# geekieo/collaborative-deep-metric-learning

Measured on NVIDIA B200. Metric: train_triplets_per_sec, higher is better.
Workload: dtype fp16 operands / fp32 accumulate (tcgen05 kind::f16), fp32 master weights

## Files before the change

collaborative-deep-metric-learning_b200/_lib.py:

```python
import ctypes
import os
from ctypes import POINTER, c_char_p, c_float, c_int, c_int32, c_int64, c_void_p

_HERE = os.path.dirname(os.path.abspath(__file__))
LIB_PATH = os.path.join(_HERE, "libcdml.so")

F16, BF16 = 0, 1
EPI_STORE_F32, EPI_STORE_16, EPI_L2NORM, EPI_MASK_LEAKY, EPI_MASK_BITS = 0, 1, 2, 3, 4
METRIC_L2, METRIC_IP = 0, 1

_P = c_void_p
_SIGNATURES = {
  "cdml_ctx_create": (c_int, [c_int, POINTER(c_void_p)]),
  "cdml_ctx_destroy": (c_int, [_P]),
  "cdml_last_error": (c_char_p, []),
  "cdml_version": (c_int, []),
  "cdml_ctx_poll_errors": (c_int, [_P, _P, POINTER(c_int32)]),
  "cdml_gather_rows": (c_int, [_P, _P, c_int64, c_int64, c_int64, _P, c_int, c_int64, _P, c_int64, _P]),
  "cdml_rows_normalize_cast": (c_int, [_P, _P, c_int64, c_int64, c_int64, c_int, c_float, _P, c_int64, c_int, _P,
                                       c_int64, _P, _P]),
  "cdml_gemm16": (c_int, [_P, _P, c_int, c_int64, _P, c_int, c_int64, c_int64, c_int64, c_int64, c_int, c_int, _P,
                          c_int64, _P, c_float, _P, _P, c_int64, c_int, c_int64, POINTER(c_int), _P]),
  "cdml_gemm16_auto_splits": (c_int, [_P, c_int64, c_int64, c_int64]),
  "cdml_sum_partials": (c_int, [_P, _P, c_int, c_int64, c_int64, c_float, _P, _P]),
  "cdml_colsum_workspace_floats": (c_int64, [c_int64, c_int64]),
  "cdml_colsum16": (c_int, [_P, _P, c_int64, c_int64, c_int64, c_int, _P, _P, _P]),
  "cdml_triplet_hinge": (c_int, [_P, _P, c_int64, c_int, c_int64, _P, c_float, c_float, _P, c_float, _P, _P, _P, _P,
                                 _P, _P, c_int64, c_int, _P, _P]),
  "cdml_adam_prepare": (c_int, [_P, _P, c_float, c_float, c_float, c_int, c_float, c_float, _P, _P]),
  "cdml_adam_apply": (c_int, [_P, _P, _P, _P, _P, c_int64, _P, c_float, c_float, c_float, c_float, _P, c_int, _P]),
  "cdml_opt_workspace_floats": (c_int64, []),
  "cdml_opt_sumsq": (c_int, [_P, _P, _P, c_int64, c_float, c_float, _P, _P, _P]),
  "cdml_opt_apply": (c_int, [_P, c_int, _P, _P, _P, _P, c_int64, _P, _P, c_float, c_float, c_float, c_float, c_float,
                             c_float, c_float, c_float, c_float, _P, c_int, _P]),
  "cdml_ew16": (c_int, [_P, c_int, _P, c_int64, _P, c_int64, _P, c_int64, _P, c_int64, c_int64, c_int, c_float, c_int, _P]),
  "cdml_rows_l2norm16": (c_int, [_P, _P, c_int64, c_int, c_int64, c_float, c_int, _P, c_int64, _P, _P, c_int64, _P]),
  "cdml_desim_workspace_bytes": (c_int64, [c_int64, c_int, c_int]),
  "cdml_desim": (c_int, [_P, _P, c_int64, c_int, c_int64, _P, _P, c_int64, c_int, c_int64, c_int64, c_float, c_int, _P, _P,
                         c_int64, c_int64, _P]),
  "cdml_desim_simple": (c_int, [_P, _P, c_int64, c_int, c_int64, _P, c_int, c_int64, _P, c_int64, _P]),
  "cdml_sample_triplets": (c_int, [_P, _P, c_int64, c_int64, c_int64, c_int64, ctypes.c_uint64, _P, _P]),
  "cdml_format_knn_rows": (c_int64, [_P, _P, c_int64, c_int, c_int64, c_int64, _P, _P, c_int64, _P, c_int64]),
  "cdml_format_f32": (c_int64, [_P, c_int64, _P, c_int64]),
  "cdml_parse_features_txt": (c_int64, [_P, c_int64, c_int, _P, c_int64, _P, _P, c_int]),
  "cdml_cast16": (c_int, [_P, _P, c_int64, _P, c_int, _P]),
  "cdml_fill_column16": (c_int, [_P, _P, c_int64, c_int64, c_int64, c_float, c_int, _P]),
  "cdml_mine_semihard": (c_int, [_P, _P, c_int64, c_int, _P, c_int64, _P, c_int64, c_int, c_float, _P, _P, _P]),
  "cdml_mine_distance_weighted": (c_int, [_P, _P, c_int64, c_int, _P, c_int64, _P, c_int64, c_int, c_float, c_float,
                                          ctypes.c_uint64, _P, _P, _P, _P]),
  "cdml_mine_last_stats": (c_int, [_P, _P, _P]),
  "cdml_knn_index_build": (c_int, [_P, _P, c_int64, c_int, c_int64, c_int, _P, POINTER(c_void_p)]),
  "cdml_knn_index_destroy": (c_int, [_P]),
  "cdml_knn_search": (c_int, [_P, _P, _P, c_int64, c_int64, c_int, _P, _P, c_int64, _P]),
  "cdml_knn_bounds": (c_int, [_P, _P, _P, c_int64, c_int64, c_int, c_int, _P, _P, _P]),
  "cdml_knn_search_bounded": (c_int, [_P, _P, _P, c_int64, c_int64, c_int, _P, _P, _P, _P, c_int64, _P]),
  "cdml_knn_last_stats": (c_int, [_P, POINTER(c_int64)]),
  "cdml_knn_merge": (c_int, [_P, _P, _P, c_int, c_int64, c_int, c_int, _P, _P, _P]),
  "cdml_knn_shard_bounds": (c_int, [_P, _P, _P, c_int64, c_int64, c_int, c_int, _P, _P]),
  "cdml_knn_shard_collect": (c_int, [_P, _P, _P, c_int64, c_int64, c_int, c_int, _P, _P, _P]),
  "cdml_knn_shard_refine": (c_int, [_P, _P, _P, c_int64, c_int64, c_int, _P, _P, c_int64, _P, _P]),
  "cdml_knn_merge_packed": (c_int, [_P, _P, c_int, c_int64, c_int, c_int, _P, _P, _P, _P]),
  "cdml_knn_unpack_records": (c_int, [_P, _P, c_int64, c_int, _P, _P, _P]),
  "cdml_mean_pair_dist": (c_int, [_P, _P, c_int64, c_int, _P, c_int64, _P, _P]),
# ... 56 lines not shown
```

collaborative-deep-metric-learning_b200/csrc/rowops.cu:

```cuda
#include <algorithm>
#include "../../include/cdml.h"
#include "ctx.cuh"

namespace cdml {

constexpr int kWarpsPerBlock = 8;
constexpr int kRowThreads = kWarpsPerBlock * 32;

__device__ __forceinline__ float warp_sum(float v) {
#pragma unroll
  for (int o = 16; o > 0; o >>= 1) v += __shfl_xor_sync(0xffffffffu, v, o);
  return v;
}

static inline int row_grid(cdml_ctx* ctx, int64_t rows) {
  const int64_t blocks = (rows + kWarpsPerBlock - 1) / kWarpsPerBlock;
  const int64_t cap = static_cast<int64_t>(ctx->num_sms) * 8;
  return static_cast<int>(blocks < cap ? (blocks > 0 ? blocks : 1) : cap);
}

template <typename IdxT, typename VecT>
__global__ void __launch_bounds__(kRowThreads)
gather_rows_kernel(const uint8_t* __restrict__ table, int64_t num_rows, int64_t row_bytes, int64_t pitch,
                   const IdxT* __restrict__ idx, int64_t n, uint8_t* __restrict__ out, int64_t out_pitch,
// ... 312 lines not shown
  __syncthreads();
  {
    float t = 0.f;
#pragma unroll
    for (int w = 0; w < kWarpsPerBlock; ++w) t += sh[w][threadIdx.x];
    const int64_t c = static_cast<int64_t>(blockIdx.x) * kColStripV + threadIdx.x;
    if (c < N) partial[static_cast<int64_t>(blockIdx.y) * N + c] = t;
  }
}

__global__ void sum_partials_kernel(const float* __restrict__ parts, int num_parts, int64_t stride, int64_t n,
                                    float scale, float* __restrict__ out) {
  for (int64_t i = static_cast<int64_t>(blockIdx.x) * blockDim.x + threadIdx.x; i < n;
       i += static_cast<int64_t>(gridDim.x) * blockDim.x) {
    float t = 0.f;
    for (int s = 0; s < num_parts; ++s) t += parts[s * stride + i];
    out[i] = t * scale;
  }
}

__global__ void sum_partials_vec4_kernel(const float4* __restrict__ parts, int num_parts, int64_t stride4, int64_t n4,
                                         float scale, float4* __restrict__ out) {
  for (int64_t i = static_cast<int64_t>(blockIdx.x) * blockDim.x + threadIdx.x; i < n4;
       i += static_cast<int64_t>(gridDim.x) * blockDim.x) {
    float4 t = make_float4(0.f, 0.f, 0.f, 0.f);
    for (int s = 0; s < num_parts; ++s) {
      const float4 v = __ldg(parts + s * stride4 + i);
      t.x += v.x, t.y += v.y, t.z += v.z, t.w += v.w;
    }
    out[i] = make_float4(t.x * scale, t.y * scale, t.z * scale, t.w * scale);
  }
}

__global__ void adam_prepare_kernel(int64_t* step, float base_lr, float decay_steps, float decay_rate, int staircase,
                                    float beta1, float beta2, float* scalars) {
  const int64_t gs = *step;
  const double t = static_cast<double>(gs + 1);
  double p = static_cast<double>(gs) / static_cast<double>(decay_steps);
  if (staircase) p = floor(p);
  const double lr = static_cast<double>(base_lr) * pow(static_cast<double>(decay_rate), p);
  const double lr_t = lr * sqrt(1.0 - pow(static_cast<double>(beta2), t)) / (1.0 - pow(static_cast<double>(beta1), t));
  scalars[0] = static_cast<float>(lr_t);
  scalars[1] = static_cast<float>(lr);
  scalars[2] = static_cast<float>(t);
  scalars[3] = 0.f;
  *step = gs + 1;
}

template <int kBf16>
__global__ void adam_apply_kernel(float* __restrict__ w, float* __restrict__ m, float* __restrict__ v,
                                  const float* __restrict__ g, int64_t n, const float* __restrict__ scalars,
                                  float beta1, float beta2, float eps, float gscale, uint16_t* __restrict__ w16) {
  const float lr_t = scalars[0];
  for (int64_t i = static_cast<int64_t>(blockIdx.x) * blockDim.x + threadIdx.x; i < n;
       i += static_cast<int64_t>(gridDim.x) * blockDim.x) {
    const float gi = g[i] * gscale;
    const float mi = beta1 * m[i] + (1.f - beta1) * gi;
    const float vi = beta2 * v[i] + (1.f - beta2) * gi * gi;
    const float wi = w[i] - lr_t * mi / (sqrtf(vi) + eps);
    m[i] = mi, v[i] = vi, w[i] = wi;
    if (w16 != nullptr) w16[i] = static_cast<uint16_t>(pack2<kBf16>(wi, 0.f));
  }
}

__global__ void fill_column16_kernel(uint16_t* __restrict__ X, int64_t rows, int64_t ld, int64_t col, uint16_t bits) {
  for (int64_t r = static_cast<int64_t>(blockIdx.x) * blockDim.x + threadIdx.x; r < rows;
       r += static_cast<int64_t>(gridDim.x) * blockDim.x)
    X[r * ld + col] = bits;
}

template <int kBf16>
__global__ void cast16_kernel(const float* __restrict__ in, int64_t n, uint16_t* __restrict__ out) {
  for (int64_t i = static_cast<int64_t>(blockIdx.x) * blockDim.x + threadIdx.x; i < n;
       i += static_cast<int64_t>(gridDim.x) * blockDim.x)
    out[i] = static_cast<uint16_t>(pack2<kBf16>(in[i], 0.f));
}

__global__ void __launch_bounds__(kRowThreads)
pair_dist_kernel(const float* __restrict__ V, int64_t ld, int D, const int64_t* __restrict__ pairs, int64_t P,
                 float* __restrict__ dist) {
  const int warp = threadIdx.x >> 5, lane = threadIdx.x & 31;
  for (int64_t i = static_cast<int64_t>(blockIdx.x) * kWarpsPerBlock + warp; i < P;
       i += static_cast<int64_t>(gridDim.x) * kWarpsPerBlock) {
    const float* a = V + pairs[2 * i] * ld;
    const float* b = V + pairs[2 * i + 1] * ld;
    float s = 0.f;
    for (int j = lane; j < D; j += 32) {
      const float d = a[j] - b[j];
      s = fmaf(d, d, s);
    }
    s = warp_sum(s);
    if (lane == 0) dist[i] = s;
  }
}
// ... 296 lines not shown
                                                                         stride / 4, n / 4, scale,
                                                                         reinterpret_cast<float4*>(out));
  else
    sum_partials_kernel<<<flat_grid(ctx, n, 256), 256, 0, st>>>(parts, num_parts, stride, n, scale, out);
  CDML_CHECK_CUDA(cudaGetLastError());
  return 0;
}

int cdml_adam_prepare(cdml_ctx* ctx, int64_t* step_counter, float base_lr, float decay_steps, float decay_rate,
                      int staircase, float beta1, float beta2, float* scalars, void* stream) {
  CDML_REQUIRE(ctx && step_counter && scalars, "cdml_adam_prepare: NULL argument");
  adam_prepare_kernel<<<1, 1, 0, static_cast<cudaStream_t>(stream)>>>(step_counter, base_lr, decay_steps, decay_rate,
                                                                      staircase, beta1, beta2, scalars);
  CDML_CHECK_CUDA(cudaGetLastError());
  return 0;
}

int cdml_adam_apply(cdml_ctx* ctx, float* w, float* m, float* v, const float* g, int64_t n, const float* scalars,
                    float beta1, float beta2, float eps, float grad_scale, void* w16, int dtype16, void* stream) {
  CDML_REQUIRE(ctx && w && m && v && g && scalars, "cdml_adam_apply: NULL argument");
  if (n == 0) return 0;
  cudaStream_t st = static_cast<cudaStream_t>(stream);
  const int grid = flat_grid(ctx, n, 256);
  if (dtype16 == CDML_BF16)
    adam_apply_kernel<1><<<grid, 256, 0, st>>>(w, m, v, g, n, scalars, beta1, beta2, eps, grad_scale,
                                               static_cast<uint16_t*>(w16));
  else
    adam_apply_kernel<0><<<grid, 256, 0, st>>>(w, m, v, g, n, scalars, beta1, beta2, eps, grad_scale,
                                               static_cast<uint16_t*>(w16));
  CDML_CHECK_CUDA(cudaGetLastError());
  return 0;
}

int64_t cdml_opt_workspace_floats(void) { return 2 * kSumsqBlocks + 2; }

int cdml_opt_sumsq(cdml_ctx* ctx, const float* g, const float* w, int64_t n, float grad_scale, float wd_reg,
                   float* workspace, float* out2, void* stream) {
  CDML_REQUIRE(ctx && g && w && workspace && out2 && n >= 0, "cdml_opt_sumsq: bad argument");
  cudaStream_t st = static_cast<cudaStream_t>(stream);
  const int blocks = static_cast<int>(std::max<int64_t>(1, std::min<int64_t>((n + 255) / 256, kSumsqBlocks)));
  opt_sumsq_stage1_kernel<<<blocks, 256, 0, st>>>(g, w, n, grad_scale, wd_reg, workspace);
  opt_sumsq_stage2_kernel<<<1, 32, 0, st>>>(workspace, blocks, out2);
  CDML_CHECK_CUDA(cudaGetLastError());
  return 0;
}

int cdml_opt_apply(cdml_ctx* ctx, int kind, float* w, float* m, float* v, const float* g, int64_t n, const float* scalars,
                   const float* norms, float beta1, float beta2, float eps, float grad_scale, float wd_reg, float clip_norm,
                   float momentum, float lars_weight_decay, float lars_eeta, void* w16, int dtype16, void* stream) {
  CDML_REQUIRE(ctx && w && g && scalars && kind >= 0 && kind <= 3, "cdml_opt_apply: bad argument");
  CDML_REQUIRE(kind != 0 || (m && v), "cdml_opt_apply: Adam needs m and v");
  CDML_REQUIRE((kind != 1 && kind != 2) || m, "cdml_opt_apply: momentum optimizers need the accumulator m");
  CDML_REQUIRE((clip_norm <= 0.f && kind != 2) || norms, "cdml_opt_apply: clipping / LARS need the norms of cdml_opt_sumsq");
  if (n == 0) return 0;
  cudaStream_t st = static_cast<cudaStream_t>(stream);
  const int grid = flat_grid(ctx, n, 256);
  if (dtype16 == CDML_BF16)
    opt_apply_kernel<1><<<grid, 256, 0, st>>>(kind, w, m, v, g, n, scalars, norms, beta1, beta2, eps, grad_scale, wd_reg,
                                              clip_norm, momentum, lars_weight_decay, lars_eeta, static_cast<uint16_t*>(w16));
  else
    opt_apply_kernel<0><<<grid, 256, 0, st>>>(kind, w, m, v, g, n, scalars, norms, beta1, beta2, eps, grad_scale, wd_reg,
                                              clip_norm, momentum, lars_weight_decay, lars_eeta, static_cast<uint16_t*>(w16));
  CDML_CHECK_CUDA(cudaGetLastError());
  return 0;
}

// ... 102 lines not shown
```

collaborative-deep-metric-learning_b200/engine.py:

```python
import math
import os
import weakref

import numpy as np
import torch

from . import ops
from ._lib import BF16, EPI_L2NORM, EPI_MASK_BITS, EPI_MASK_LEAKY, EPI_STORE_16, EPI_STORE_F32, F16

LEAKY_ALPHA = 0.2


def _pad8(n):
  return (n + 7) // 8 * 8


def _pad64(n):
  return (n + 63) // 64 * 64


class TowerEngine:

  def __init__(self, dims, device=None, dtype16=F16, seed=2, bias_init=0.0, base_lr=1e-3, margin=0.8,
               lr_decay_steps=1000000, lr_decay=0.96, beta1=0.9, beta2=0.999, eps=1e-8, alpha=LEAKY_ALPHA,
               process_group=None, init_params=None, optimizer="adam", clip_norm=0.0, reg_penalty=0.0, l2_penalty=1e-8,
               momentum=0.9, lars_weight_decay=1e-4, lars_eeta=1e-3, layer_shapes=None):
    if not torch.cuda.is_available():
      raise RuntimeError("TowerEngine needs a CUDA device (sm_100a); there is no CPU path")
    self.device = torch.device(device if device is not None else "cuda:%d" % torch.cuda.current_device())
    self.dims = [int(d) for d in dims]
    if self.dims[-1] > 256:
      raise ValueError("output_size must be <= 256 (the L2-norm epilogue holds the whole row in one tile)")
    for d in self.dims[1:]:
      if d % 8:
        raise ValueError("layer widths must be multiples of 8 (16-byte row pitch for TMA); got %d" % d)
    self.shapes = [(int(a), int(b)) for a, b in (layer_shapes if layer_shapes is not None else zip(self.dims[:-1], self.dims[1:]))]
    for _, d in self.shapes:
      if d % 8:
        raise ValueError("layer widths must be multiples of 8 (16-byte row pitch for TMA); got %d" % d)
    self.L = len(self.shapes)
    self.dtype16 = dtype16
    self.t16 = ops.TORCH16[dtype16]
    self.alpha = float(alpha)
    self.margin = float(margin)
    self.base_lr, self.lr_decay_steps, self.lr_decay = float(base_lr), float(lr_decay_steps), float(lr_decay)
    self.beta1, self.beta2, self.eps = beta1, beta2, eps
    self.opt_kind = {"adam": ops.OPT_ADAM, "momentum": ops.OPT_MOMENTUM, "lars": ops.OPT_LARS, "sgd": ops.OPT_SGD}[optimizer]
    self.clip_norm, self.wd_reg = float(clip_norm), float(reg_penalty) * float(l2_penalty)
    self.momentum, self.lars_wd, self.lars_eeta = float(momentum), float(lars_weight_decay), float(lars_eeta)
    self.pg = process_group
    self.world = torch.distributed.get_world_size(process_group) if process_group is not None else 1
    self.F = self.dims[0]
    self.F_pad = _pad64(self.F + 1)
    self.loss_scale = 1.0
    self.fused_bias_grad = True
    self.ddp_buckets = os.environ.get("CDML_DDP_BUCKETS", "0") == "1"
    self._ones_checked = {}

    sizes = []
    for fi, fo in self.shapes:
      sizes += [fi * fo, fo]
    self.offsets = np.concatenate([[0], np.cumsum(sizes)]).astype(np.int64)
    self.offsets = np.concatenate([[0], np.cumsum([_pad8(s) for s in sizes])]).astype(np.int64)
    total = int(self.offsets[-1])
    dev = self.device
    self.w = torch.zeros(total, dtype=torch.float32, device=dev)
    self.m = torch.zeros(total, dtype=torch.float32, device=dev)
    self.v = torch.zeros(total, dtype=torch.float32, device=dev)
    self.g = torch.zeros(total, dtype=torch.float32, device=dev)
    self.sizes = sizes
    self.W = [self._view(self.w, 2 * l).view(*self.shapes[l]) for l in range(self.L)]
    self.b = [self._view(self.w, 2 * l + 1) for l in range(self.L)]
    self.gW = [self._view(self.g, 2 * l).view(*self.shapes[l]) for l in range(self.L)]
    self.gb = [self._view(self.g, 2 * l + 1) for l in range(self.L)]
    self.W16 = [torch.zeros(self.shapes[l], dtype=self.t16, device=dev) for l in range(self.L)]
    self.step_counter = torch.zeros(1, dtype=torch.int64, device=dev)
    self.dw_cutoff, self.dw_seed = 0.5, int(seed)
    self.scalars = torch.zeros(4, dtype=torch.float32, device=dev)
    self.norms = torch.zeros((2 * self.L, 2), dtype=torch.float32, device=dev)
    self.opt_ws = torch.empty((ops.opt_workspace_floats(),), dtype=torch.float32, device=dev)
    self._bufs = {}
    self._pinned_bufs = set()
    self._ws = {}

    if init_params is None:
      rng = np.random.RandomState(seed)
      init_params = []
      biases = list(bias_init) if isinstance(bias_init, (list, tuple)) else [bias_init] * self.L
      for (fi, fo), b0 in zip(self.shapes, biases):
        lim = math.sqrt(6.0 / (fi + fo))
        init_params.append((rng.uniform(-lim, lim, size=(fi, fo)).astype(np.float32), np.full((fo,), b0, np.float32)))
    self.load_params(init_params)

  def _view(self, flat, i):
    o = int(self.offsets[i])
    return flat[o:o + self.sizes[i]]

  def load_params(self, params):
    for l, (W, b) in enumerate(params):
      self.W[l].copy_(torch.as_tensor(np.asarray(W), dtype=torch.float32))
      self.b[l].copy_(torch.as_tensor(np.asarray(b), dtype=torch.float32))
    self.refresh_shadows()

  def refresh_shadows(self):
    for l in range(self.L):
      ops.cast16(self.W[l], self.W16[l])

  def get_params(self):
    return [(self.W[l].detach().cpu().numpy().copy(), self.b[l].detach().cpu().numpy().copy()) for l in range(self.L)]

  OPT_NAMES = {ops.OPT_ADAM: "adam", ops.OPT_MOMENTUM: "momentum", ops.OPT_LARS: "lars", ops.OPT_SGD: "sgd"}
# ... 24 lines not shown
    return int(self.step_counter.item())

  def _buffers(self, R, train):
    key = (R, train)
    buf = self._bufs.get(key)
    if buf is not None:
      if key not in self._pinned_bufs:
        self._bufs[key] = self._bufs.pop(key)
      return buf
    dev, t16 = self.device, self.t16
    D = self.dims[-1]
    def mat16(cols, spare=0):
      return torch.empty((R, _pad64(cols + spare)), dtype=t16, device=dev)[:, :cols]

    def act16(cols):
      m = mat16(cols, 1 if train else 0)
      if train and self._bias_row_ok(cols, m.stride(0)):
        ops.fill_column16(m, cols, 1.0)
      return m

    buf = {"acts": [act16(self.dims[l + 1]) for l in range(self.L - 1)],
           "e": torch.empty((R, D), dtype=torch.float32, device=dev),
           "rinv": torch.empty((R,), dtype=torch.float32, device=dev)}
    if train:
      B = R // 3
      buf["dz"] = [mat16(self.dims[l + 1]) for l in range(self.L)]
      buf["mask"] = [ops.sign_mask_buffer(R, self.dims[l + 1], dev) for l in range(self.L - 1)]
      buf["G"] = torch.empty((R, D), dtype=torch.float32, device=dev)
      buf["loss"] = {k: torch.empty((B,), dtype=torch.float32, device=dev) for k in ("pos_dist", "neg_dist", "hinge_dist")}
      buf["loss"]["stats"] = torch.empty((4,), dtype=torch.float32, device=dev)
      in_pitch = [self.F_pad] + [a.stride(0) for a in buf["acts"]]
      buf["wrows"] = [self.dims[l] + (1 if self._bias_row_ok(self.dims[l], in_pitch[l]) else 0) for l in range(self.L)]
      buf["splits"] = [ops.auto_splits(self.w, buf["wrows"][l], self.dims[l + 1], R) for l in range(self.L)]
      part = max(s * buf["wrows"][l] * self.dims[l + 1] if s > 1 else 0 for l, s in enumerate(buf["splits"]))
      buf["partials"] = torch.empty((max(part, 1),), dtype=torch.float32, device=dev)
      buf["colsum_ws"] = torch.empty((max(ops.colsum_workspace_floats(R, d) for d in self.dims[1:]),),
                                     dtype=torch.float32, device=dev)
    self._store_buffers(key, buf)
    return buf

  def _store_buffers(self, key, buf):
    self._bufs[key] = buf
    loose = [k for k in self._bufs if k not in self._pinned_bufs]
    for k in loose[:max(0, len(loose) - 4)]:
      del self._bufs[k]

  def _bias_row_ok(self, width, pitch):
    return self.fused_bias_grad and pitch > width

  def forward_rows(self, x16, R, train=False, want_e16=None):
    buf = self._buffers(R, train)
    h = x16
    for l in range(self.L):
      K, N = self.dims[l], self.dims[l + 1]
      if l < self.L - 1:
        ops.gemm16(h, self.W16[l], R, N, K, 0, 1, EPI_STORE_16, buf["acts"][l], bias=self.b[l], alpha=self.alpha,
                   aux0=buf["mask"][l] if train else None)
        h = buf["acts"][l]
      else:
        ops.gemm16(h, self.W16[l], R, N, K, 0, 1, EPI_L2NORM, buf["e"], bias=self.b[l], alpha=self.alpha,
                   aux0=buf["rinv"], aux1=want_e16)
    return buf

  def embed(self, x, batch_rows=None):
    n = x.shape[0]
    x16, _, _ = ops.rows_normalize_cast(x, self.dtype16, 1, 1e-12, ld_out=self.F_pad)
    buf = self.forward_rows(x16, n, train=False)
    return buf["e"]
# ... 46 lines not shown
    self.backward_rows(x16, R, buf, input_ones)
    self.apply_gradients(B)
    return buf["loss"]["stats"]

  def _mine_negatives(self, e16, e, guid, B, mine):
    if mine is True or mine == "semihard":
      return ops.mine_semihard(e16, e, guid, B, self.margin, want_dist=False)[0]
    if mine == "distance_weighted":
      return ops.mine_distance_weighted(e16, e, guid, B, self.margin, self.dw_cutoff, self.dw_seed, self.step_counter,
                                        want_dist=False)[0]
    raise ValueError("mine must be False, True, 'semihard' or 'distance_weighted' (got %r)" % (mine,))

  def backward_rows(self, x16, R, buf, input_ones=False):
    dz = buf["dz"]
    self._pending = []
    for l in range(self.L - 1, -1, -1):
      K_in, N_out = self.dims[l], self.dims[l + 1]
      inp = x16 if l == 0 else buf["acts"][l - 1]
      self._weight_gradient(l, inp, dz[l], R, buf, with_bias_row=(l > 0 or input_ones))
      if self.world > 1 and self.ddp_buckets and l > 0:
        o0, o1 = int(self.offsets[2 * l]), int(self.offsets[2 * l + 2])
        self._pending.append(torch.distributed.all_reduce(self.g[o0:o1], group=self.pg, async_op=True))
      if l > 0:
        ops.gemm16(dz[l], self.W16[l], R, K_in, N_out, 0, 0, EPI_MASK_BITS, dz[l - 1], alpha=self.alpha,
                   aux1=buf["mask"][l - 1])

  def _weight_gradient(self, l, inp, dz, R, buf, with_bias_row):
    K_in, N_out = self.shapes[l]
    s = buf["splits"][l]
    rows = buf["wrows"][l] if with_bias_row else K_in
    o = int(self.offsets[2 * l])
    gWb = self.g[o:o + rows * N_out]
    if s > 1:
      used = ops.gemm16(inp, dz, rows, N_out, R, 1, 1, EPI_STORE_F32, buf["partials"], num_splits=s,
                        split_stride=rows * N_out, ld_out=N_out)
      ops.sum_partials(buf["partials"], used, rows * N_out, rows * N_out, gWb)
    else:
      ops.gemm16(inp, dz, rows, N_out, R, 1, 1, EPI_STORE_F32, gWb, ld_out=N_out)
    if rows == K_in:
      ops.colsum16(dz, R, N_out, self.gb[l], buf["colsum_ws"])

  def apply_gradients(self, B_local):
    if self.world > 1:
      pending = getattr(self, "_pending", [])
      if pending:
        torch.distributed.all_reduce(self.g[:int(self.offsets[2])], group=self.pg)
        for w in pending:
          w.wait()
        self._pending = []
      else:
        torch.distributed.all_reduce(self.g, group=self.pg)
    ops.adam_prepare(self.step_counter, self.scalars, self.base_lr, self.lr_decay_steps, self.lr_decay, True,
                     self.beta1, self.beta2)
    scale = 1.0 / (B_local * self.world * self.loss_scale)
    plain_adam = self.opt_kind == ops.OPT_ADAM and self.clip_norm <= 0 and self.wd_reg == 0
    for l in range(self.L):
      for i, (w, g, w16, wd) in enumerate(((self.W[l], self.gW[l], self.W16[l], self.wd_reg), (self.b[l], self.gb[l], None, 0.0))):
        m, v = self._view(self.m, 2 * l + i), self._view(self.v, 2 * l + i)
        if plain_adam:
          ops.adam_apply(w, m, v, g, self.scalars, self.beta1, self.beta2, self.eps, scale, w16=w16)
          continue
        norms = None
        if self.clip_norm > 0 or self.opt_kind == ops.OPT_LARS:
          norms = ops.opt_sumsq(g, w, self.norms[2 * l + i], self.opt_ws, grad_scale=scale, wd_reg=wd)
        ops.opt_apply(self.opt_kind, w, m, v, g, self.scalars, norms, self.beta1, self.beta2,
                      0.0 if self.opt_kind == ops.OPT_LARS else self.eps, scale, wd, self.clip_norm, self.momentum,
                      self.lars_wd, self.lars_eeta, w16=w16)

  def reg_loss(self):
    tot = 0.0
    for l in range(self.L):
      ops.opt_sumsq(self.gW[l], self.W[l], self.norms[2 * l], self.opt_ws)
      tot += 0.5 * float(self.norms[2 * l][1].item())
    return tot * (self.wd_reg if self.wd_reg else 0.0)

  def capture_step(self, table16, B, mine=False):
    if self.world > 1 and os.environ.get("CDML_DDP_GRAPH", "1") == "0":
      raise RuntimeError("capture_step disabled for data-parallel runs (CDML_DDP_GRAPH=0)")
    G = self._table_rows(table16)
    ar = torch.arange(B, dtype=torch.int64, device=self.device)
    static_idx = torch.stack([(3 * ar) % G, (3 * ar + 1) % G, (3 * ar + 2) % G], dim=1).contiguous()
    snap = (self.w.clone(), self.m.clone(), self.v.clone(), self.step_counter.clone())
    side = torch.cuda.Stream(device=self.device)
    side.wait_stream(torch.cuda.current_stream())
    with torch.cuda.stream(side):
      for _ in range(2):
        self.train_step_indices(table16, static_idx, mine=mine)
    torch.cuda.current_stream().wait_stream(side)
    torch.cuda.synchronize()
    if self.world > 1:
      torch.distributed.barrier(group=self.pg)
    graph = torch.cuda.CUDAGraph()
    launches0 = ops.launch_count()
    with torch.cuda.graph(graph, capture_error_mode="thread_local" if self.world > 1 else "global"):
      stats = self.train_step_indices(table16, static_idx, mine=mine)
    launches_per_step = ops.launch_count() - launches0
    ops._count(-launches_per_step)
    self.w.copy_(snap[0]), self.m.copy_(snap[1]), self.v.copy_(snap[2]), self.step_counter.copy_(snap[3])
    self.refresh_shadows()
    torch.cuda.synchronize()
# ... 16 lines not shown
```

collaborative-deep-metric-learning_b200/fusion.py:

```python
import json

import torch

from . import ops
from ._lib import EPI_L2NORM, EPI_MASK_BITS, EPI_MASK_LEAKY, EPI_STORE_16, F16
from .engine import LEAKY_ALPHA, TowerEngine, _pad64


def _widths(spec):
  w = []
  for e in spec:
    if e["op"] == "input":
      w.append(int(e["hi"]) - int(e["lo"]))
    elif e["op"] == "fc":
      w.append(int(e["out"]))
    elif e["op"] in ("mul", "add"):
      w.append(w[e["src"][0]])
    else:
      w.append(w[e["src"]])
  return w


class GraphEngine(TowerEngine):

  def __init__(self, spec, feature_size=None, device=None, dtype16=F16, seed=2, init_params=None, loss_scale=256.0, **kw):
    spec = [dict(e) for e in spec]
    if not spec or spec[-1]["op"] != "l2norm" or any(e["op"] == "l2norm" for e in spec[:-1]):
      raise ValueError("the op list must end with its only l2norm (the model output)")
    self.spec = spec
    self.widths = _widths(spec)
    for i, e in enumerate(spec):
      srcs = e["src"] if isinstance(e.get("src"), list) else [e["src"]] if "src" in e else []
      if any(not (0 <= s < i) for s in srcs):
        raise ValueError("op %d consumes a later op" % i)
      if any(spec[s]["op"] == "input" for s in srcs) and e["op"] != "fc":
        raise NotImplementedError("input slices feed fully_connected layers only")
      if e["op"] in ("mul", "add") and len({self.widths[s] for s in srcs}) != 1:
        raise ValueError("op %d joins tensors of different widths" % i)
      if e["op"] == "mul" and len(srcs) != 2:
# ... 48 lines not shown

  def _buffers(self, R, train):
    key = (R, train)
    buf = self._bufs.get(key)
    if buf is not None:
      if key not in self._pinned_bufs:
        self._bufs[key] = self._bufs.pop(key)
      return buf
    dev, t16, spec, D = self.device, self.t16, self.spec, self.widths[-1]

    def mat16(cols, ones):
      m = torch.empty((R, _pad64(cols + 1)), dtype=t16, device=dev)
      if ones:
        ops.fill_column16(m, cols, 1.0)
      return m[:, :cols]

    buf = {"val": {}, "e": torch.empty((R, D), dtype=torch.float32, device=dev),
           "rinv": torch.empty((R,), dtype=torch.float32, device=dev)}
    for i, e in enumerate(spec[:-1]):
      if e["op"] != "input" and i != self.fused_out:
        feeds_fc = any(spec[c]["op"] == "fc" for c in self.consumers[i])
        buf["val"][i] = mat16(self.widths[i], train and feeds_fc)
    if train:
      B = R // 3
      buf["mask"] = {s: ops.sign_mask_buffer(R, self.widths[s], dev) for s in self._masked_nodes()}
      buf["dz"] = {i: mat16(self.widths[i], False) for i in self.fcs}
      buf["grad"] = {}
      buf["dzo"] = mat16(D, False)
      buf["G"] = torch.empty((R, D), dtype=torch.float32, device=dev)
      buf["loss"] = {k: torch.empty((B,), dtype=torch.float32, device=dev) for k in ("pos_dist", "neg_dist", "hinge_dist")}
      buf["loss"]["stats"] = torch.empty((4,), dtype=torch.float32, device=dev)
      buf["wrows"] = [fi + 1 for fi, _ in self.shapes]
      buf["splits"] = [ops.auto_splits(self.w, buf["wrows"][l], fo, R) for l, (_, fo) in enumerate(self.shapes)]
      part = max(s * buf["wrows"][l] * self.shapes[l][1] if s > 1 else 0 for l, s in enumerate(buf["splits"]))
      buf["partials"] = torch.empty((max(part, 1),), dtype=torch.float32, device=dev)
      buf["colsum_ws"] = torch.empty((max(ops.colsum_workspace_floats(R, fo) for _, fo in self.shapes),),
                                     dtype=torch.float32, device=dev)
    self._store_buffers(key, buf)
    return buf

  def _masked_nodes(self):
    spec = self.spec
    return [e["src"] for i, e in enumerate(spec) if e["op"] == "fc" and spec[e["src"]]["op"] == "fc"
            and len(self.consumers[e["src"]]) == 1 and e["src"] != self.fused_out]

  def _scratch(self, buf, key, cols):
    m = buf["grad"].get(key)
    if m is None:
      R = buf["e"].shape[0]
      m = buf["grad"][key] = torch.empty((R, _pad64(cols + 1)), dtype=self.t16, device=self.device)[:, :cols]
    return m

  def forward_rows(self, xsegs, R, train=False, want_e16=None):
    buf = self._buffers(R, train)
    val = dict(buf["val"])
    for k, i in enumerate(self.inputs):
      val[i] = xsegs[k][:, :self.widths[i]]
    for i, e in enumerate(self.spec):
      op = e["op"]
      if op == "fc":
        l = self.layer_of[i]
        K, N = self.shapes[l]
        if i == self.fused_out:
          ops.gemm16(val[e["src"]], self.W16[l], R, N, K, 0, 1, EPI_L2NORM, buf["e"], bias=self.b[l], alpha=self.alpha,
                     aux0=buf["rinv"], aux1=want_e16)
        else:
          ops.gemm16(val[e["src"]], self.W16[l], R, N, K, 0, 1, EPI_STORE_16, val[i], bias=self.b[l], alpha=self.alpha,
                     aux0=buf["mask"].get(i) if train else None)
# ... 126 lines not shown
```

collaborative-deep-metric-learning_b200/ops.py:

```python
import ctypes

import torch

from . import _lib
from ._lib import BF16, EPI_L2NORM, EPI_MASK_BITS, EPI_MASK_LEAKY, EPI_STORE_16, EPI_STORE_F32, F16, check, ptr, stream_ptr

TORCH16 = {F16: torch.float16, BF16: torch.bfloat16}

_LAUNCHES = 0


def _count(n):
  global _LAUNCHES
  _LAUNCHES += n


def launch_count():
  return _LAUNCHES


def _ctx(t):
  return _lib.context(t.device.index if t.device.index is not None else torch.cuda.current_device())


# ... 101 lines not shown
  pos = out.get("pos_dist") if "pos_dist" in out else torch.empty((B,), dtype=torch.float32, device=dev)
  neg = out.get("neg_dist") if "neg_dist" in out else torch.empty((B,), dtype=torch.float32, device=dev)
  hin = out.get("hinge_dist") if "hinge_dist" in out else torch.empty((B,), dtype=torch.float32, device=dev)
  stats = out.get("stats") if "stats" in out else torch.empty((4,), dtype=torch.float32, device=dev)
  dE = None
  if want_dE:
    dE = out.get("dE") if "dE" in out else torch.empty_like(E)
  if dz16 is not None and dE is None and workspace is None:
    workspace = torch.empty((3 * B * E.stride(0),), dtype=torch.float32, device=dev)
  mined_grad = neg_row is not None and (dE is not None or dz16 is not None)
  _count(2 + (2 if mined_grad else 0) + (1 if dz16 is not None else 0))
  check(_lib.load().cdml_triplet_hinge(_ctx(E), ptr(E), B, D, E.stride(0), ptr(neg_row), float(margin), float(grad_scale),
                                       ptr(rinv), float(leaky_alpha), ptr(pos), ptr(neg), ptr(hin), ptr(stats), ptr(dE),
                                       ptr(dz16), dz16.stride(0) if dz16 is not None else 0,
                                       dtype16_of(dz16) if dz16 is not None else F16, ptr(workspace), stream_ptr()))
  return {"pos_dist": pos, "neg_dist": neg, "hinge_dist": hin, "stats": stats, "dE": dE, "dz16": dz16}


def adam_prepare(step_counter, scalars, base_lr, decay_steps=1e6, decay_rate=0.96, staircase=True, beta1=0.9,
                 beta2=0.999):
  _count(1)
  check(_lib.load().cdml_adam_prepare(_ctx(scalars), ptr(step_counter), float(base_lr), float(decay_steps),
                                      float(decay_rate), int(staircase), float(beta1), float(beta2), ptr(scalars),
                                      stream_ptr()))


def adam_apply(w, m, v, g, scalars, beta1=0.9, beta2=0.999, eps=1e-8, grad_scale=1.0, w16=None):
  _count(1)
  check(_lib.load().cdml_adam_apply(_ctx(w), ptr(w), ptr(m), ptr(v), ptr(g), w.numel(), ptr(scalars), float(beta1),
                                    float(beta2), float(eps), float(grad_scale), ptr(w16),
                                    dtype16_of(w16) if w16 is not None else F16, stream_ptr()))


OPT_ADAM, OPT_MOMENTUM, OPT_LARS, OPT_SGD = 0, 1, 2, 3


def opt_workspace_floats():
  return int(_lib.load().cdml_opt_workspace_floats())


def opt_sumsq(g, w, out2, workspace, grad_scale=1.0, wd_reg=0.0):
  _count(2)
  check(_lib.load().cdml_opt_sumsq(_ctx(w), ptr(g), ptr(w), w.numel(), float(grad_scale), float(wd_reg), ptr(workspace),
                                   ptr(out2), stream_ptr()))
  return out2


def opt_apply(kind, w, m, v, g, scalars, norms=None, beta1=0.9, beta2=0.999, eps=1e-8, grad_scale=1.0, wd_reg=0.0,
              clip_norm=0.0, momentum=0.9, lars_weight_decay=1e-4, lars_eeta=1e-3, w16=None):
  _count(1)
  check(_lib.load().cdml_opt_apply(_ctx(w), int(kind), ptr(w), ptr(m), ptr(v), ptr(g), w.numel(), ptr(scalars), ptr(norms),
                                   float(beta1), float(beta2), float(eps), float(grad_scale), float(wd_reg), float(clip_norm),
                                   float(momentum), float(lars_weight_decay), float(lars_eeta), ptr(w16),
                                   dtype16_of(w16) if w16 is not None else F16, stream_ptr()))


EW_MUL, EW_ADD, EW_MUL_ADD_BOTH, EW_MASK, EW_MUL_ADD, EW_FMA, EW_MUL_ADD_MASK, EW_MUL_MASK = 0, 1, 2, 3, 4, 5, 6, 7


def ew16(op, a, b, out, c=None, alpha=0.2):
  rows, cols = out.shape
  _count(1)
  check(_lib.load().cdml_ew16(_ctx(out), int(op), ptr(a), a.stride(0), ptr(b), b.stride(0), ptr(c),
                              c.stride(0) if c is not None else 0, ptr(out), out.stride(0), rows, cols, float(alpha),
                              dtype16_of(out), stream_ptr()))
  return out
# ... 239 lines not shown
```

include/cdml.h:

```cpp
#ifndef CDML_H_
#define CDML_H_
#include <stdint.h>

#ifdef __cplusplus
extern "C" {
#endif

typedef struct cdml_ctx cdml_ctx;

#define CDML_F16 0
#define CDML_BF16 1

int cdml_ctx_create(int device, cdml_ctx** out);
int cdml_ctx_destroy(cdml_ctx* ctx);
const char* cdml_last_error(void);
int cdml_version(void);
int cdml_ctx_poll_errors(cdml_ctx* ctx, void* stream, int32_t* flags);

int cdml_gather_rows(cdml_ctx* ctx, const void* table, int64_t num_rows, int64_t row_bytes, int64_t table_pitch_bytes,
                     const void* idx, int idx_is_64, int64_t n_idx, void* out, int64_t out_pitch_bytes, void* stream);

int cdml_rows_normalize_cast(cdml_ctx* ctx, const float* in, int64_t n, int64_t F, int64_t ld_in, int normalize,
                             float eps, void* out16, int64_t ld_out, int dtype16, float* out32, int64_t ld_out32,
                             float* sumsq, void* stream);

int cdml_gemm16(cdml_ctx* ctx, const void* A, int a_mn_major, int64_t lda, const void* B, int b_mn_major, int64_t ldb,
                int64_t M, int64_t N, int64_t K, int dtype16, int epilogue, void* out, int64_t ld_out,
                const float* bias, float alpha, void* aux0, void* aux1, int64_t ld_aux1, int num_splits,
                int64_t split_stride, int* splits_used, void* stream);
int cdml_gemm16_auto_splits(cdml_ctx* ctx, int64_t M, int64_t N, int64_t K);

int cdml_sum_partials(cdml_ctx* ctx, const float* parts, int num_parts, int64_t stride, int64_t n, float scale,
                      float* out, void* stream);

int64_t cdml_colsum_workspace_floats(int64_t R, int64_t N);
int cdml_colsum16(cdml_ctx* ctx, const void* X, int64_t R, int64_t N, int64_t ld, int dtype16, float* workspace,
                  float* out, void* stream);

int cdml_triplet_hinge(cdml_ctx* ctx, const float* E, int64_t B, int D, int64_t ld_e, const int32_t* neg_row,
                       float margin, float grad_scale, const float* rinv, float leaky_alpha, float* pos_dist,
                       float* neg_dist, float* hinge_dist, float* stats, float* dE, void* dz16, int64_t ld_dz,
                       int dtype16, float* workspace, void* stream);

int cdml_adam_prepare(cdml_ctx* ctx, int64_t* step_counter, float base_lr, float decay_steps, float decay_rate,
                      int staircase, float beta1, float beta2, float* scalars, void* stream);
int cdml_adam_apply(cdml_ctx* ctx, float* w, float* m, float* v, const float* g, int64_t n, const float* scalars,
                    float beta1, float beta2, float eps, float grad_scale, void* w16, int dtype16, void* stream);
int64_t cdml_opt_workspace_floats(void);
int cdml_opt_sumsq(cdml_ctx* ctx, const float* g, const float* w, int64_t n, float grad_scale, float wd_reg,
                   float* workspace, float* out2, void* stream);
int cdml_opt_apply(cdml_ctx* ctx, int kind, float* w, float* m, float* v, const float* g, int64_t n, const float* scalars,
                   const float* norms, float beta1, float beta2, float eps, float grad_scale, float wd_reg, float clip_norm,
                   float momentum, float lars_weight_decay, float lars_eeta, void* w16, int dtype16, void* stream);
int cdml_ew16(cdml_ctx* ctx, int op, const void* a, int64_t lda, const void* b, int64_t ldb, const void* c, int64_t ldc,
              void* out, int64_t ldo, int64_t rows, int cols, float alpha, int dtype16, void* stream);
int cdml_rows_l2norm16(cdml_ctx* ctx, const void* y16, int64_t n, int D, int64_t ld_y, float eps, int dtype16, float* e,
                       int64_t ld_e, float* rinv, void* e16, int64_t ld_e16, void* stream);
int cdml_cast16(cdml_ctx* ctx, const float* in, int64_t n, void* out16, int dtype16, void* stream);

int cdml_fill_column16(cdml_ctx* ctx, void* X16, int64_t rows, int64_t ld, int64_t col, float value, int dtype16,
                       void* stream);

int cdml_mine_semihard(cdml_ctx* ctx, const void* E16, int64_t ld16, int dtype16, const float* E32, int64_t ld32,
                       const int64_t* guid, int64_t B, int D, float margin, int32_t* neg_row, float* d_an,
                       void* stream);
int cdml_mine_distance_weighted(cdml_ctx* ctx, const void* E16, int64_t ld16, int dtype16, const float* E32,
                                int64_t ld32, const int64_t* guid, int64_t B, int D, float margin, float cutoff,
                                uint64_t seed, const int64_t* step, int32_t* neg_row, float* d_an, void* stream);
int cdml_mine_last_stats(cdml_ctx* ctx, int64_t* out2, void* stream);

typedef struct cdml_index cdml_index;
int cdml_knn_index_build(cdml_ctx* ctx, const float* X, int64_t N, int d, int64_t ldx, int metric, void* stream,
                         cdml_index** out);
int cdml_knn_index_destroy(cdml_index* index);
int cdml_knn_search(cdml_ctx* ctx, cdml_index* index, const float* Q, int64_t nq, int64_t ldq, int k, float* D,
                    int64_t* I, int64_t id_offset, void* stream);
int cdml_knn_bounds(cdml_ctx* ctx, cdml_index* index, const float* Q, int64_t nq, int64_t ldq, int k_full, int k_part,
                    float* bound_full, float* bound_part, void* stream);
int cdml_knn_search_bounded(cdml_ctx* ctx, cdml_index* index, const float* Q, int64_t nq, int64_t ldq, int k,
                            const float* bound_full, const float* bound_part, float* D, int64_t* I, int64_t id_offset,
// ... 41 lines not shown
```

Measured before the change: 5.946 million.

## Fuse Adam schedule, split-K partial reduction and all tensor updates into one multi-tensor kernel

Replaces the separate adam_prepare launch and the per-tensor adam_apply launches with a single multi-tensor Adam kernel. The kernel computes the LR schedule itself, and the last block to finish (tracked through an atomic counter) advances the step. Split-K weight-gradient partials are no longer reduced by a sum_partials launch; the optimizer kernel sums them while it updates, and each layer now gets its own offset in the partials buffer so the deferred partials stay valid. The aim is to cut kernel launches and one read-write round trip of the gradient. In exchange the code adds a grid-wide atomic completion protocol and a larger partials buffer.

```diff
diff --git a/collaborative-deep-metric-learning_b200/_lib.py b/collaborative-deep-metric-learning_b200/_lib.py
--- a/collaborative-deep-metric-learning_b200/_lib.py
+++ b/collaborative-deep-metric-learning_b200/_lib.py
@@ -29,6 +29,8 @@
                                  _P, _P, c_int64, c_int, _P, _P]),
   "cdml_adam_prepare": (c_int, [_P, _P, c_float, c_float, c_float, c_int, c_float, c_float, _P, _P]),
   "cdml_adam_apply": (c_int, [_P, _P, _P, _P, _P, c_int64, _P, c_float, c_float, c_float, c_float, _P, c_int, _P]),
+  "cdml_adam_step": (c_int, [_P, c_int, _P, _P, _P, _P, _P, _P, _P, _P, _P, c_int, _P, c_float, c_float, c_float, c_int,
+                             c_float, c_float, c_float, c_float, _P, _P, _P]),
   "cdml_opt_workspace_floats": (c_int64, []),
   "cdml_opt_sumsq": (c_int, [_P, _P, _P, c_int64, c_float, c_float, _P, _P, _P]),
   "cdml_opt_apply": (c_int, [_P, c_int, _P, _P, _P, _P, c_int64, _P, _P, c_float, c_float, c_float, c_float, c_float,
diff --git a/collaborative-deep-metric-learning_b200/csrc/rowops.cu b/collaborative-deep-metric-learning_b200/csrc/rowops.cu
--- a/collaborative-deep-metric-learning_b200/csrc/rowops.cu
+++ b/collaborative-deep-metric-learning_b200/csrc/rowops.cu
@@ -368,18 +368,37 @@
   }
 }
 
-__global__ void adam_prepare_kernel(int64_t* step, float base_lr, float decay_steps, float decay_rate, int staircase,
-                                    float beta1, float beta2, float* scalars) {
-  const int64_t gs = *step;
+struct AdamSchedule {
+  float lr_t, lr, t;
+};
+
+__device__ __forceinline__ AdamSchedule adam_schedule(int64_t gs, float base_lr, float decay_steps, float decay_rate,
+                                                      int staircase, float beta1, float beta2) {
   const double t = static_cast<double>(gs + 1);
   double p = static_cast<double>(gs) / static_cast<double>(decay_steps);
   if (staircase) p = floor(p);
   const double lr = static_cast<double>(base_lr) * pow(static_cast<double>(decay_rate), p);
   const double lr_t = lr * sqrt(1.0 - pow(static_cast<double>(beta2), t)) / (1.0 - pow(static_cast<double>(beta1), t));
-  scalars[0] = static_cast<float>(lr_t);
-  scalars[1] = static_cast<float>(lr);
-  scalars[2] = static_cast<float>(t);
-  scalars[3] = 0.f;
+  return {static_cast<float>(lr_t), static_cast<float>(lr), static_cast<float>(t)};
+}
+
+__device__ __forceinline__ void adam_store_scalars(float* scalars, const AdamSchedule& s) {
+  scalars[0] = s.lr_t, scalars[1] = s.lr, scalars[2] = s.t, scalars[3] = 0.f;
+}
+
+__device__ __forceinline__ float adam_update(float g, float gscale, float beta1, float beta2, float eps, float lr_t,
+                                             float& w, float& m, float& v) {
+  const float gi = __fmul_rn(g, gscale);
+  m = __fmaf_rn(m, beta1, __fmul_rn(1.f - beta1, gi));
+  v = __fmaf_rn(v, beta2, __fmul_rn(__fmul_rn(1.f - beta2, gi), gi));
+  w = __fsub_rn(w, __fdiv_rn(__fmul_rn(lr_t, m), __fadd_rn(__fsqrt_rn(v), eps)));
+  return w;
+}
+
+__global__ void adam_prepare_kernel(int64_t* step, float base_lr, float decay_steps, float decay_rate, int staircase,
+                                    float beta1, float beta2, float* scalars) {
+  const int64_t gs = *step;
+  adam_store_scalars(scalars, adam_schedule(gs, base_lr, decay_steps, decay_rate, staircase, beta1, beta2));
   *step = gs + 1;
 }
 
@@ -390,12 +409,98 @@
   const float lr_t = scalars[0];
   for (int64_t i = static_cast<int64_t>(blockIdx.x) * blockDim.x + threadIdx.x; i < n;
        i += static_cast<int64_t>(gridDim.x) * blockDim.x) {
-    const float gi = g[i] * gscale;
-    const float mi = beta1 * m[i] + (1.f - beta1) * gi;
-    const float vi = beta2 * v[i] + (1.f - beta2) * gi * gi;
-    const float wi = w[i] - lr_t * mi / (sqrtf(vi) + eps);
+    float wi = w[i], mi = m[i], vi = v[i];
+    adam_update(g[i], gscale, beta1, beta2, eps, lr_t, wi, mi, vi);
     m[i] = mi, v[i] = vi, w[i] = wi;
     if (w16 != nullptr) w16[i] = static_cast<uint16_t>(pack2<kBf16>(wi, 0.f));
+  }
+}
+
+constexpr int kAdamMaxTensors = 16;
+struct AdamTensor {
+  float *w, *m, *v, *g;
+  uint16_t* w16;
+  const float* parts;
+  int64_t n, stride;
+  int num_parts, vec;
+};
+struct AdamBatch {
+  AdamTensor t[kAdamMaxTensors];
+  int count;
+};
+
+constexpr int kAdamBlocksPerSm = 6;
+template <int kBf16>
+__global__ void __launch_bounds__(256, kAdamBlocksPerSm)
+adam_multi_kernel(AdamBatch batch, int64_t* __restrict__ step, float base_lr, float decay_steps, float decay_rate,
+                  int staircase, float beta1, float beta2, float eps, float gscale, int finish, float* __restrict__ scalars,
+                  unsigned int* __restrict__ done) {
+  __shared__ int64_t s_gs;
+  __shared__ float s_lr_t;
+  if (threadIdx.x == 0) {
+    s_gs = *step;
+    s_lr_t = adam_schedule(s_gs, base_lr, decay_steps, decay_rate, staircase, beta1, beta2).lr_t;
+  }
+  __syncthreads();
+  const float lr_t = s_lr_t;
+  const int64_t first = static_cast<int64_t>(blockIdx.x) * blockDim.x + threadIdx.x;
+  const int64_t stride_all = static_cast<int64_t>(gridDim.x) * blockDim.x;
+  for (int k = 0; k < batch.count; ++k) {
+    const AdamTensor& T = batch.t[k];
+    if (T.vec) {
+      float4* w4 = reinterpret_cast<float4*>(T.w);
+      float4* m4 = reinterpret_cast<float4*>(T.m);
+      float4* v4 = reinterpret_cast<float4*>(T.v);
+      float4* g4 = reinterpret_cast<float4*>(T.g);
+      const float4* p4 = reinterpret_cast<const float4*>(T.parts);
+      const int64_t n4 = T.n / 4, s4 = T.stride / 4;
+      for (int64_t i = first; i < n4; i += stride_all) {
+        float4 g;
+        if (p4 != nullptr) {
+          g = make_float4(0.f, 0.f, 0.f, 0.f);
+          for (int s = 0; s < T.num_parts; ++s) {
+            const float4 p = __ldg(p4 + s * s4 + i);
+            g.x = __fadd_rn(g.x, p.x), g.y = __fadd_rn(g.y, p.y), g.z = __fadd_rn(g.z, p.z), g.w = __fadd_rn(g.w, p.w);
+          }
+          g4[i] = g;
+        } else {
+          g = g4[i];
+        }
+        float4 w = w4[i], m = m4[i], v = v4[i];
+        adam_update(g.x, gscale, beta1, beta2, eps, lr_t, w.x, m.x, v.x);
+        adam_update(g.y, gscale, beta1, beta2, eps, lr_t, w.y, m.y, v.y);
+        adam_update(g.z, gscale, beta1, beta2, eps, lr_t, w.z, m.z, v.z);
+        adam_update(g.w, gscale, beta1, beta2, eps, lr_t, w.w, m.w, v.w);
+        w4[i] = w, m4[i] = m, v4[i] = v;
+        if (T.w16 != nullptr)
+          reinterpret_cast<uint2*>(T.w16)[i] = make_uint2(pack2<kBf16>(w.x, w.y), pack2<kBf16>(w.z, w.w));
+      }
+    } else {
+      for (int64_t i = first; i < T.n; i += stride_all) {
+        float g;
+        if (T.parts != nullptr) {
+          g = 0.f;
+          for (int s = 0; s < T.num_parts; ++s) g = __fadd_rn(g, __ldg(T.parts + s * T.stride + i));
+          T.g[i] = g;
+        } else {
+          g = T.g[i];
+        }
+        float w = T.w[i], m = T.m[i], v = T.v[i];
+        adam_update(g, gscale, beta1, beta2, eps, lr_t, w, m, v);
+        T.w[i] = w, T.m[i] = m, T.v[i] = v;
+        if (T.w16 != nullptr) T.w16[i] = static_cast<uint16_t>(pack2<kBf16>(w, 0.f));
+      }
+    }
+  }
+  if (!finish) return;
+  __syncthreads();
+  if (threadIdx.x == 0) {
+    __threadfence();
+    if (atomicAdd(done, 1u) == gridDim.x - 1) {
+      adam_store_scalars(scalars, adam_schedule(s_gs, base_lr, decay_steps, decay_rate, staircase, beta1, beta2));
+      *step = s_gs + 1;
+      *done = 0u;
+    }
   }
 }
 
@@ -758,6 +863,47 @@
   return 0;
 }
 
+int cdml_adam_step(cdml_ctx* ctx, int count, float* const* w, float* const* m, float* const* v, float* const* g,
+                   void* const* w16, const float* const* parts, const int* num_parts, const int64_t* part_stride,
+                   const int64_t* n, int dtype16, int64_t* step_counter, float base_lr, float decay_steps,
+                   float decay_rate, int staircase, float beta1, float beta2, float eps, float grad_scale, float* scalars,
+                   unsigned int* done, void* stream) {
+  CDML_REQUIRE(ctx && count >= 1 && w && m && v && g && w16 && parts && num_parts && part_stride && n && step_counter &&
+               scalars && done, "cdml_adam_step: NULL argument");
+  cudaStream_t st = static_cast<cudaStream_t>(stream);
+  int64_t total = 0;
+  for (int i = 0; i < count; ++i) {
+    CDML_REQUIRE(w[i] && m[i] && v[i] && g[i] && n[i] >= 0, "cdml_adam_step: bad tensor %d", i);
+    CDML_REQUIRE(parts[i] == nullptr || (num_parts[i] >= 1 && part_stride[i] >= n[i]),
+                 "cdml_adam_step: bad partials of tensor %d", i);
+    total += n[i];
+  }
+  const int grid = std::min(flat_grid(ctx, total / 4 + 1, 256), kAdamBlocksPerSm * ctx->num_sms);
+  for (int b = 0; b < count; b += kAdamMaxTensors) {
+    AdamBatch batch{};
+    batch.count = std::min(count - b, kAdamMaxTensors);
+    for (int k = 0; k < batch.count; ++k) {
+      const int i = b + k;
+      const uintptr_t a16 = reinterpret_cast<uintptr_t>(w[i]) | reinterpret_cast<uintptr_t>(m[i]) |
+                            reinterpret_cast<uintptr_t>(v[i]) | reinterpret_cast<uintptr_t>(g[i]) |
+                            reinterpret_cast<uintptr_t>(parts[i]);
+      const bool vec = (a16 & 15) == 0 && (reinterpret_cast<uintptr_t>(w16[i]) & 7) == 0 && n[i] % 4 == 0 &&
+                       (parts[i] == nullptr || part_stride[i] % 4 == 0);
+      batch.t[k] = AdamTensor{w[i], m[i], v[i], g[i], static_cast<uint16_t*>(w16[i]), parts[i], n[i],
+                              parts[i] != nullptr ? part_stride[i] : 0, parts[i] != nullptr ? num_parts[i] : 0, vec ? 1 : 0};
+    }
+    const int finish = b + kAdamMaxTensors >= count ? 1 : 0;
+    if (dtype16 == CDML_BF16)
+      adam_multi_kernel<1><<<grid, 256, 0, st>>>(batch, step_counter, base_lr, decay_steps, decay_rate, staircase, beta1,
+                                                 beta2, eps, grad_scale, finish, scalars, done);
+    else
+      adam_multi_kernel<0><<<grid, 256, 0, st>>>(batch, step_counter, base_lr, decay_steps, decay_rate, staircase, beta1,
+                                                 beta2, eps, grad_scale, finish, scalars, done);
+    CDML_CHECK_CUDA(cudaGetLastError());
+  }
+  return 0;
+}
+
 int64_t cdml_opt_workspace_floats(void) { return 2 * kSumsqBlocks + 2; }
 
 int cdml_opt_sumsq(cdml_ctx* ctx, const float* g, const float* w, int64_t n, float grad_scale, float wd_reg,
diff --git a/collaborative-deep-metric-learning_b200/engine.py b/collaborative-deep-metric-learning_b200/engine.py
--- a/collaborative-deep-metric-learning_b200/engine.py
+++ b/collaborative-deep-metric-learning_b200/engine.py
@@ -13,6 +13,14 @@
 
 def _pad8(n):
   return (n + 7) // 8 * 8
+
+
+def partial_offsets(splits, rows, cols):
+  offs, tot = [], 0
+  for s, r, c in zip(splits, rows, cols):
+    offs.append(tot)
+    tot += _pad8(s * r * c) if s > 1 else 0
+  return offs, max(tot, 1)
 
 
 def _pad64(n):
@@ -77,6 +85,8 @@
     self.step_counter = torch.zeros(1, dtype=torch.int64, device=dev)
     self.dw_cutoff, self.dw_seed = 0.5, int(seed)
     self.scalars = torch.zeros(4, dtype=torch.float32, device=dev)
+    self.adam_done = torch.zeros(1, dtype=torch.int32, device=dev)
+    self._deferred = {}
     self.norms = torch.zeros((2 * self.L, 2), dtype=torch.float32, device=dev)
     self.opt_ws = torch.empty((ops.opt_workspace_floats(),), dtype=torch.float32, device=dev)
     self._bufs = {}
@@ -167,8 +177,8 @@
       in_pitch = [self.F_pad] + [a.stride(0) for a in buf["acts"]]
       buf["wrows"] = [self.dims[l] + (1 if self._bias_row_ok(self.dims[l], in_pitch[l]) else 0) for l in range(self.L)]
       buf["splits"] = [ops.auto_splits(self.w, buf["wrows"][l], self.dims[l + 1], R) for l in range(self.L)]
-      part = max(s * buf["wrows"][l] * self.dims[l + 1] if s > 1 else 0 for l, s in enumerate(buf["splits"]))
-      buf["partials"] = torch.empty((max(part, 1),), dtype=torch.float32, device=dev)
+      buf["part_off"], part = partial_offsets(buf["splits"], buf["wrows"], self.dims[1:])
+      buf["partials"] = torch.empty((part,), dtype=torch.float32, device=dev)
       buf["colsum_ws"] = torch.empty((max(ops.colsum_workspace_floats(R, d) for d in self.dims[1:]),),
                                      dtype=torch.float32, device=dev)
     self._store_buffers(key, buf)
@@ -281,9 +291,13 @@
     o = int(self.offsets[2 * l])
     gWb = self.g[o:o + rows * N_out]
     if s > 1:
-      used = ops.gemm16(inp, dz, rows, N_out, R, 1, 1, EPI_STORE_F32, buf["partials"], num_splits=s,
+      parts = buf["partials"][buf["part_off"][l]:]
+      used = ops.gemm16(inp, dz, rows, N_out, R, 1, 1, EPI_STORE_F32, parts, num_splits=s,
                         split_stride=rows * N_out, ld_out=N_out)
-      ops.sum_partials(buf["partials"], used, rows * N_out, rows * N_out, gWb)
+      if self._plain_adam() and self.world == 1 and (rows == K_in or int(self.offsets[2 * l + 1]) == o + K_in * N_out):
+        self._deferred[l] = (parts, used, rows * N_out, rows > K_in)
+      else:
+        ops.sum_partials(parts, used, rows * N_out, rows * N_out, gWb)
     else:
       ops.gemm16(inp, dz, rows, N_out, R, 1, 1, EPI_STORE_F32, gWb, ld_out=N_out)
     if rows == K_in:
@@ -299,22 +313,33 @@
         self._pending = []
       else:
         torch.distributed.all_reduce(self.g, group=self.pg)
+    scale = 1.0 / (B_local * self.world * self.loss_scale)
+    if self._plain_adam():
+      tensors = []
+      for l in range(self.L):
+        d = self._deferred.pop(l, None)
+        for i, (w, g, w16) in enumerate(((self.W[l], self.gW[l], self.W16[l]), (self.b[l], self.gb[l], None))):
+          parts, num, stride = None, 0, 0
+          if d is not None and (i == 0 or d[3]):
+            parts, num, stride = d[0][i * self.sizes[2 * l]:], d[1], d[2]
+          tensors.append((w, self._view(self.m, 2 * l + i), self._view(self.v, 2 * l + i), g, w16, parts, num, stride))
+      ops.adam_step(tensors, self.step_counter, self.scalars, self.adam_done, self.base_lr, self.lr_decay_steps,
+                    self.lr_decay, True, self.beta1, self.beta2, self.eps, scale)
+      return
     ops.adam_prepare(self.step_counter, self.scalars, self.base_lr, self.lr_decay_steps, self.lr_decay, True,
                      self.beta1, self.beta2)
-    scale = 1.0 / (B_local * self.world * self.loss_scale)
-    plain_adam = self.opt_kind == ops.OPT_ADAM and self.clip_norm <= 0 and self.wd_reg == 0
     for l in range(self.L):
       for i, (w, g, w16, wd) in enumerate(((self.W[l], self.gW[l], self.W16[l], self.wd_reg), (self.b[l], self.gb[l], None, 0.0))):
         m, v = self._view(self.m, 2 * l + i), self._view(self.v, 2 * l + i)
-        if plain_adam:
-          ops.adam_apply(w, m, v, g, self.scalars, self.beta1, self.beta2, self.eps, scale, w16=w16)
-          continue
         norms = None
         if self.clip_norm > 0 or self.opt_kind == ops.OPT_LARS:
           norms = ops.opt_sumsq(g, w, self.norms[2 * l + i], self.opt_ws, grad_scale=scale, wd_reg=wd)
         ops.opt_apply(self.opt_kind, w, m, v, g, self.scalars, norms, self.beta1, self.beta2,
                       0.0 if self.opt_kind == ops.OPT_LARS else self.eps, scale, wd, self.clip_norm, self.momentum,
                       self.lars_wd, self.lars_eeta, w16=w16)
+
+  def _plain_adam(self):
+    return self.opt_kind == ops.OPT_ADAM and self.clip_norm <= 0 and self.wd_reg == 0
 
   def reg_loss(self):
     tot = 0.0
diff --git a/collaborative-deep-metric-learning_b200/fusion.py b/collaborative-deep-metric-learning_b200/fusion.py
--- a/collaborative-deep-metric-learning_b200/fusion.py
+++ b/collaborative-deep-metric-learning_b200/fusion.py
@@ -4,7 +4,7 @@
 
 from . import ops
 from ._lib import EPI_L2NORM, EPI_MASK_BITS, EPI_MASK_LEAKY, EPI_STORE_16, F16
-from .engine import LEAKY_ALPHA, TowerEngine, _pad64
+from .engine import LEAKY_ALPHA, TowerEngine, _pad64, partial_offsets
 
 
 def _widths(spec):
@@ -119,8 +119,8 @@
       buf["loss"]["stats"] = torch.empty((4,), dtype=torch.float32, device=dev)
       buf["wrows"] = [fi + 1 for fi, _ in self.shapes]
       buf["splits"] = [ops.auto_splits(self.w, buf["wrows"][l], fo, R) for l, (_, fo) in enumerate(self.shapes)]
-      part = max(s * buf["wrows"][l] * self.shapes[l][1] if s > 1 else 0 for l, s in enumerate(buf["splits"]))
-      buf["partials"] = torch.empty((max(part, 1),), dtype=torch.float32, device=dev)
+      buf["part_off"], part = partial_offsets(buf["splits"], buf["wrows"], [fo for _, fo in self.shapes])
+      buf["partials"] = torch.empty((part,), dtype=torch.float32, device=dev)
       buf["colsum_ws"] = torch.empty((max(ops.colsum_workspace_floats(R, fo) for _, fo in self.shapes),),
                                      dtype=torch.float32, device=dev)
     self._store_buffers(key, buf)
diff --git a/collaborative-deep-metric-learning_b200/ops.py b/collaborative-deep-metric-learning_b200/ops.py
--- a/collaborative-deep-metric-learning_b200/ops.py
+++ b/collaborative-deep-metric-learning_b200/ops.py
@@ -157,6 +157,21 @@
                                     dtype16_of(w16) if w16 is not None else F16, stream_ptr()))
 
 
+def adam_step(tensors, step_counter, scalars, done, base_lr, decay_steps=1e6, decay_rate=0.96, staircase=True, beta1=0.9,
+              beta2=0.999, eps=1e-8, grad_scale=1.0):
+  k = len(tensors)
+  arr = lambda ts: (ctypes.c_void_p * k)(*[None if t is None else t.data_ptr() for t in ts])
+  w, m, v, g, w16, parts, nparts, stride = zip(*tensors)
+  dtype16 = next((dtype16_of(t) for t in w16 if t is not None), F16)
+  _count((k + 15) // 16)
+  check(_lib.load().cdml_adam_step(_ctx(scalars), k, arr(w), arr(m), arr(v), arr(g), arr(w16), arr(parts),
+                                   (ctypes.c_int * k)(*[int(s) for s in nparts]),
+                                   (ctypes.c_int64 * k)(*[int(s) for s in stride]),
+                                   (ctypes.c_int64 * k)(*[t.numel() for t in w]), dtype16, ptr(step_counter),
+                                   float(base_lr), float(decay_steps), float(decay_rate), int(staircase), float(beta1),
+                                   float(beta2), float(eps), float(grad_scale), ptr(scalars), ptr(done), stream_ptr()))
+
+
 OPT_ADAM, OPT_MOMENTUM, OPT_LARS, OPT_SGD = 0, 1, 2, 3
 
 
diff --git a/include/cdml.h b/include/cdml.h
--- a/include/cdml.h
+++ b/include/cdml.h
@@ -46,6 +46,11 @@
                       int staircase, float beta1, float beta2, float* scalars, void* stream);
 int cdml_adam_apply(cdml_ctx* ctx, float* w, float* m, float* v, const float* g, int64_t n, const float* scalars,
                     float beta1, float beta2, float eps, float grad_scale, void* w16, int dtype16, void* stream);
+int cdml_adam_step(cdml_ctx* ctx, int count, float* const* w, float* const* m, float* const* v, float* const* g,
+                   void* const* w16, const float* const* parts, const int* num_parts, const int64_t* part_stride,
+                   const int64_t* n, int dtype16, int64_t* step_counter, float base_lr, float decay_steps,
+                   float decay_rate, int staircase, float beta1, float beta2, float eps, float grad_scale, float* scalars,
+                   unsigned int* done, void* stream);
 int64_t cdml_opt_workspace_floats(void);
 int cdml_opt_sumsq(cdml_ctx* ctx, const float* g, const float* w, int64_t n, float grad_scale, float wd_reg,
                    float* workspace, float* out2, void* stream);
```

New measurement: 5.929 million (median of 6 runs). No clear change (-0.3%).
